# zhenyuw16/Uni3DETR

Hardware: AMD Instinct MI355X
Metric: scenes/sec (fwd+bwd) SUN-RGB-D 20k pts, 300 queries (higher is better)
Workload: dtype bf16

## Files before the change

include/u3d_hip.h:

```cpp
#ifndef U3D_HIP_H_
#define U3D_HIP_H_

#include <stddef.h>
#include <stdint.h>

#ifdef __cplusplus
extern "C" {
#endif

typedef struct ihipStream_t* u3d_stream;

enum {
  U3D_OK = 0,
  U3D_ERR_ARG = -1,
  U3D_ERR_UNSUPPORTED = -2,
  U3D_ERR_LAUNCH = -3,
  U3D_ERR_WORKSPACE = -4
};

enum { U3D_F32 = 0, U3D_BF16 = 1 };

int32_t u3d_version(void);
const char* u3d_strerror(int32_t code);

int32_t u3d_event_create(void** event);
int32_t u3d_event_record(void* event, int32_t external, u3d_stream s);
int32_t u3d_event_elapsed_ms(void* start, void* stop, float* ms);
int32_t u3d_event_destroy(void* event);

typedef struct u3d_bitgrid {
  void* words;
  void* prefix;
  int32_t batch, dz, dy, dx;
  int32_t layout;
  int32_t row_capacity;
} u3d_bitgrid;

int64_t u3d_bitgrid_nwords(int32_t batch, int32_t dz, int32_t dy, int32_t dx);
int64_t u3d_bitgrid_nwords_layout(int32_t batch, int32_t dz, int32_t dy, int32_t dx, int32_t layout);

int32_t u3d_bitgrid_mark(const u3d_bitgrid* g, const int32_t* coors, int32_t n, u3d_stream s);

int32_t u3d_bitgrid_mark_strided(const u3d_bitgrid* g, const int32_t* in_coors, const int32_t* n_dev,
                                 int32_t n_cap, const int32_t ksize[3], const int32_t stride[3],
                                 const int32_t pad[3], u3d_stream s);

int64_t u3d_bitgrid_scan_scratch(int64_t nwords);
int32_t u3d_bitgrid_scan(const u3d_bitgrid* g, void* scratch, u3d_stream s);

int32_t u3d_bitgrid_rank(const u3d_bitgrid* g, const int32_t* coors, int32_t n, int32_t* rank, u3d_stream s);

int32_t u3d_bitgrid_coords(const u3d_bitgrid* g, int32_t* coors_out, int32_t cap, u3d_stream s);

int32_t u3d_nbr_table(const u3d_bitgrid* target, const int32_t* q_coors, const int32_t* n_dev, int32_t n_cap,
                      const int32_t ksize[3], const int32_t stride[3], const int32_t pad[3], int32_t mode,
                      int32_t* nbr, int32_t ld, u3d_stream s);

int32_t u3d_dense_nbr_table(int32_t batch, const int32_t q_dims[3], const int32_t t_dims[3], const int32_t ksize[3],
                            const int32_t stride[3], const int32_t pad[3], int32_t mode, int32_t* nbr, int32_t ld,
                            u3d_stream s);

int64_t u3d_voxelize_hard_workspace(int32_t n_total, int32_t batch, int32_t max_pts_per_scene);
int32_t u3d_voxelize_hard(const float* points, const int32_t* scene_off, int32_t batch, int32_t n_total,
                          int32_t max_pts_per_scene, int32_t nfeat, const float voxel_size[3],
                          const float pc_range[6], int32_t max_points, int32_t max_voxels,
                          float* voxels, int32_t* coors, int32_t* num_points, float* mean,
                          int32_t* voxel_off, void* workspace, int64_t workspace_bytes, u3d_stream s);

int32_t u3d_voxelize_dynamic(const float* points, const int32_t* scene_off, int32_t batch, int32_t n_total, int32_t nfeat,
                             const float voxel_size[3], const float pc_range[6], int32_t* coors, u3d_stream s);
int32_t u3d_scatter_mean(const float* points, const int32_t* rank, int32_t n_total, int32_t nfeat, float* sums,
                         int32_t* counts, int32_t n_voxels, u3d_stream s);

int32_t u3d_spconv_fwd(const void* in, const void* w, const int32_t* nbr, int32_t ld, void* out,
                       const int32_t* n_out_dev, int32_t n_out_cap, int32_t cin, int32_t cout, int32_t kvol,
                       int32_t transpose_w, int32_t dtype, u3d_stream s);

int32_t u3d_igemm_fwd_bf16(const void* in, const void* w, const int32_t* nbr, int32_t ld, void* out,
                           const int32_t* n_out_dev, int32_t n_out_cap, int32_t cin, int32_t cout, int32_t kvol,
                           int32_t transpose_w, u3d_stream s);
int32_t u3d_igemm_fwd_add_bf16(const void* in, const void* w, const int32_t* nbr, int32_t ld, const void* addend, void* out,
                               const int32_t* n_out_dev, int32_t n_out_cap, int32_t cin, int32_t cout, int32_t kvol,
                               int32_t transpose_w, u3d_stream s);
int32_t u3d_linear_bf16(const void* x, const void* w, const float* bias, int32_t relu, void* out, const int32_t* m_dev,
                        int32_t m_cap, int32_t k, int32_t n, u3d_stream s);
int64_t u3d_bn_fold_job_bytes(void);
int32_t u3d_bn_fold_job_blocks(int32_t kvol, int32_t cout, int32_t cin);
int32_t u3d_bn_fold_batched(const void* jobs, int32_t njobs, int32_t total_blocks, u3d_stream s);
int32_t u3d_igemm_fwd_affine_bf16(const void* in, const void* w_folded, const int32_t* nbr, int32_t ld, const float* shift, int32_t relu,
                                  void* out, const int32_t* n_out_dev, int32_t n_out_cap, int32_t cin, int32_t cout, int32_t kvol,
                                  u3d_stream s);
int32_t u3d_igemm_fwd_affine_plan(int32_t n_out_cap, int32_t cin, int32_t cout, int32_t kvol, int32_t has_nbr, int32_t* kernel,
                                  int32_t* rows, int32_t* cols);
int32_t u3d_igemm_fwd_split_bf16(const void* in, const void* w, const int32_t* nbr, int32_t ld, float* out, const int32_t* n_out_dev,
                                 int32_t n_out_cap, int32_t cin, int32_t cout, int32_t kvol3, double* stats, const float* addend, u3d_stream s);
int32_t u3d_igemm_direct_split_bf16(const void* in, const void* w3, const int32_t* nbr, int32_t ld, float* out, const int32_t* n_out_dev,
                                    int32_t n_out_cap, int32_t n_in_cap, int32_t cin, int32_t cout, u3d_stream s);
int32_t u3d_igemm_direct_affine_bf16(const void* in, const void* w_folded, const int32_t* nbr, int32_t ld, const float* shift,
                                     int32_t relu, const void* addend, void* out, const int32_t* n_out_dev, int32_t n_out_cap,
                                     int32_t cin, int32_t cout, u3d_stream s);
// ... 468 lines not shown
```

uni3detr_amd/csrc/geometry.hip:

```cpp
#include "common.h"

extern "C" int64_t u3d_bitgrid_nwords(int32_t batch, int32_t dz, int32_t dy, int32_t dx) {
  return (int64_t)batch * ((dz + 3) / 4) * ((dy + 3) / 4) * ((dx + 3) / 4);
}
extern "C" int64_t u3d_bitgrid_nwords_layout(int32_t batch, int32_t dz, int32_t dy, int32_t dx, int32_t layout) {
  if (layout == 1) return ((int64_t)batch * dz * dy * dx + 63) / 64;
  return u3d_bitgrid_nwords(batch, dz, dy, dx);
}
static inline long long grid_nwords(const u3d_bitgrid* g) { return u3d_bitgrid_nwords_layout(g->batch, g->dz, g->dy, g->dx, g->layout); }

__global__ void k_bitgrid_mark(BitGridDev g, unsigned long long* words, const int4* __restrict__ coors, int n) {
  int i = blockIdx.x * blockDim.x + threadIdx.x;
  if (i >= n) return;
  int4 c = coors[i];
  if (c.x < 0 || c.x >= g.B) return;
  if ((unsigned)c.y >= (unsigned)g.Dz || (unsigned)c.z >= (unsigned)g.Dy || (unsigned)c.w >= (unsigned)g.Dx) return;
  atomicOr(&words[u3d_word_index(g, c.x, c.y, c.z, c.w)], 1ull << u3d_bit_index(g, c.x, c.y, c.z, c.w));
}

extern "C" int32_t u3d_bitgrid_mark(const u3d_bitgrid* g, const int32_t* coors, int32_t n, u3d_stream s) {
  U3D_REQUIRE(g && g->words && coors, U3D_ERR_ARG);
  if (n <= 0) return U3D_OK;
  BitGridDev d = u3d_make_grid(g);
  hipLaunchKernelGGL(k_bitgrid_mark, dim3(u3d_cdiv(n, 256)), dim3(256), 0, s, d, (unsigned long long*)g->words,
// ... 222 lines not shown
      int bit = __ffsll((long long)bits) - 1;
      bits &= bits - 1;
      long long t = w * 64 + bit;
      int x = (int)(t % g.Dx); t /= g.Dx;
      int y = (int)(t % g.Dy); t /= g.Dy;
      int z = (int)(t % g.Dz); t /= g.Dz;
      if ((int)r < cap) out[r] = make_int4((int)t, z, y, x);
      ++r;
    }
    return;
  }
  long long t = w;
  int bx = (int)(t % g.bx); t /= g.bx;
  int by = (int)(t % g.by); t /= g.by;
  int bz = (int)(t % g.bz); t /= g.bz;
  int b = (int)t;
  while (bits) {
    int bit = __ffsll((long long)bits) - 1;
    bits &= bits - 1;
    if ((int)r < cap) out[r] = make_int4(b, bz * 4 + (bit >> 4), by * 4 + ((bit >> 2) & 3), bx * 4 + (bit & 3));
    ++r;
  }
}

extern "C" int32_t u3d_bitgrid_coords(const u3d_bitgrid* g, int32_t* coors_out, int32_t cap, u3d_stream s) {
  U3D_REQUIRE(g && g->words && g->prefix && coors_out, U3D_ERR_ARG);
  long long nwords = grid_nwords(g);
  hipLaunchKernelGGL(k_bitgrid_coords, dim3(u3d_cdiv(nwords, 256)), dim3(256), 0, s, u3d_make_grid(g), nwords,
                     (int4*)coors_out, cap);
  U3D_CHECK_LAUNCH();
  return U3D_OK;
}

__global__ void k_nbr_table(BitGridDev g, const int4* __restrict__ q, const int* __restrict__ n_dev, int n_cap,
                            Conv3 cv, int mode, int* __restrict__ nbr, int ld) {
  int i = blockIdx.x * blockDim.x + threadIdx.x;
  if (i >= ld) return;
  int n = min(*n_dev, n_cap);
  int kvol = cv.k[0] * cv.k[1] * cv.k[2];
  if (i >= n) {
    for (int k = 0; k < kvol; ++k) nbr[(long long)k * ld + i] = -1;
    return;
  }
  int4 c = q[i];
  int k = 0;
  for (int kz = 0; kz < cv.k[0]; ++kz)
    for (int ky = 0; ky < cv.k[1]; ++ky)
      for (int kx = 0; kx < cv.k[2]; ++kx, ++k) {
        int r = -1;
        if (mode == 0) {
          r = u3d_grid_lookup(g, c.x, c.y * cv.s[0] - cv.p[0] + kz, c.z * cv.s[1] - cv.p[1] + ky, c.w * cv.s[2] - cv.p[2] + kx);
        } else {
          int tz = c.y + cv.p[0] - kz, ty = c.z + cv.p[1] - ky, tx = c.w + cv.p[2] - kx;
          if (tz >= 0 && ty >= 0 && tx >= 0 && tz % cv.s[0] == 0 && ty % cv.s[1] == 0 && tx % cv.s[2] == 0)
            r = u3d_grid_lookup(g, c.x, tz / cv.s[0], ty / cv.s[1], tx / cv.s[2]);
        }
        nbr[(long long)k * ld + i] = r;
      }
}

extern "C" int32_t u3d_nbr_table(const u3d_bitgrid* target, const int32_t* q_coors, const int32_t* n_dev, int32_t n_cap,
                                 const int32_t ksize[3], const int32_t stride[3], const int32_t pad[3], int32_t mode,
                                 int32_t* nbr, int32_t ld, u3d_stream s) {
  U3D_REQUIRE(target && target->words && target->prefix && q_coors && n_dev && nbr, U3D_ERR_ARG);
  U3D_REQUIRE(ld >= n_cap && (mode == 0 || mode == 1), U3D_ERR_ARG);
  if (ld <= 0) return U3D_OK;
  Conv3 cv;
  for (int i = 0; i < 3; ++i) { cv.k[i] = ksize[i]; cv.s[i] = stride[i]; cv.p[i] = pad[i]; U3D_REQUIRE(stride[i] > 0 && ksize[i] > 0, U3D_ERR_ARG); }
  hipLaunchKernelGGL(k_nbr_table, dim3(u3d_cdiv(ld, 256)), dim3(256), 0, s, u3d_make_grid(target), (const int4*)q_coors,
                     n_dev, n_cap, cv, mode, nbr, ld);
  U3D_CHECK_LAUNCH();
  return U3D_OK;
}

__global__ void k_dense_nbr_table(int B, int qz, int qy, int qx, int tz, int ty, int tx, Conv3 cv, int mode,
                                  int* __restrict__ nbr, int ld) {
  int i = blockIdx.x * blockDim.x + threadIdx.x;
  if (i >= ld) return;
  int kvol = cv.k[0] * cv.k[1] * cv.k[2];
  long long nq = (long long)B * qz * qy * qx;
  if (i >= nq) {
    for (int k = 0; k < kvol; ++k) nbr[(long long)k * ld + i] = -1;
    return;
  }
  int x = i % qx; int t = i / qx;
  int y = t % qy; t /= qy;
  int z = t % qz; int b = t / qz;
  int k = 0;
  for (int kz = 0; kz < cv.k[0]; ++kz)
    for (int ky = 0; ky < cv.k[1]; ++ky)
      for (int kx = 0; kx < cv.k[2]; ++kx, ++k) {
        int pz, py, px;
        bool ok = true;
        if (mode == 0) {
          pz = z * cv.s[0] - cv.p[0] + kz; py = y * cv.s[1] - cv.p[1] + ky; px = x * cv.s[2] - cv.p[2] + kx;
        } else {
          int uz = z + cv.p[0] - kz, uy = y + cv.p[1] - ky, ux = x + cv.p[2] - kx;
          ok = uz >= 0 && uy >= 0 && ux >= 0 && uz % cv.s[0] == 0 && uy % cv.s[1] == 0 && ux % cv.s[2] == 0;
          pz = uz / cv.s[0]; py = uy / cv.s[1]; px = ux / cv.s[2];
        }
        ok = ok && (unsigned)pz < (unsigned)tz && (unsigned)py < (unsigned)ty && (unsigned)px < (unsigned)tx;
        nbr[(long long)k * ld + i] = ok ? (int)((((long long)b * tz + pz) * ty + py) * tx + px) : -1;
      }
// ... 98 lines not shown
                           const int* __restrict__ slot_of, int* __restrict__ vid, int* __restrict__ scene_cnt) {
  __shared__ unsigned wsum[16];
  __shared__ unsigned carry_s;
  int b = blockIdx.x;
  int p0 = scene_off[b], n = scene_off[b + 1] - p0;
  long long tb = (long long)b * cfg.hsize;
  if (threadIdx.x == 0) carry_s = 0;
  __syncthreads();
  int lane = threadIdx.x & 63, wid = threadIdx.x >> 6;
  for (int base = 0; base < n; base += 1024) {
    int il = base + threadIdx.x;
    int sl = -1;
    unsigned flag = 0;
    if (il < n) {
      sl = slot_of[p0 + il];
      if (sl >= 0 && first[tb + sl] == (unsigned)il) flag = 1;
    }
    unsigned long long bal = __ballot(flag);
    unsigned in_wave = __popcll(bal & ((1ull << lane) - 1ull));
    if (lane == 0) wsum[wid] = __popcll(bal);
    __syncthreads();
    unsigned woff = 0, tot = 0;
    for (int w = 0; w < 16; ++w) { unsigned v = wsum[w]; if (w < wid) woff += v; tot += v; }
    unsigned carry = carry_s;
    if (flag) {
      unsigned r = carry + woff + in_wave;
      vid[tb + sl] = (r < (unsigned)cfg.max_voxels) ? (int)r : -1;
    }
    __syncthreads();
    if (threadIdx.x == 0) carry_s = carry + tot;
    __syncthreads();
  }
  if (threadIdx.x == 0) scene_cnt[b] = (int)min(carry_s, (unsigned)cfg.max_voxels);
}

__global__ void k_vox_offsets(const int* __restrict__ scene_cnt, int B, int* __restrict__ voxel_off) {
  if (threadIdx.x == 0 && blockIdx.x == 0) {
    int acc = 0;
    for (int b = 0; b < B; ++b) { voxel_off[b] = acc; acc += scene_cnt[b]; }
    voxel_off[B] = acc;
  }
}

__global__ void k_vox_write(const float* __restrict__ pts, const int* __restrict__ scene_off, int B, int n_total, VoxCfg cfg,
                            const unsigned* __restrict__ keys, const unsigned* __restrict__ first, const int* __restrict__ head,
                            const int* __restrict__ next, const int* __restrict__ slot_of, const int* __restrict__ vid,
                            const int* __restrict__ voxel_off, float* __restrict__ voxels, int4* __restrict__ coors,
                            int* __restrict__ num_points, float* __restrict__ mean) {
  int i = blockIdx.x * blockDim.x + threadIdx.x;
  if (i >= n_total || i >= scene_off[B]) return;
  int sl = slot_of[i];
  if (sl < 0) return;
  int b = 0;
  while (b + 1 < B && i >= scene_off[b + 1]) ++b;
  int p0 = scene_off[b];
  int il = i - p0;
  long long tb = (long long)b * cfg.hsize;
  if (first[tb + sl] != (unsigned)il) return;
  int v = vid[tb + sl];
  if (v < 0) return;
  long long row = (long long)voxel_off[b] + v;
  unsigned key = keys[tb + sl];
  int cx = (int)(key % (unsigned)cfg.grid[0]);
  unsigned t = key / (unsigned)cfg.grid[0];
  int cy = (int)(t % (unsigned)cfg.grid[1]);
  int cz = (int)(t / (unsigned)cfg.grid[1]);
// ... 2 lines not shown
  float acc[8];
  const int nf = cfg.nfeat;
  for (int f = 0; f < 8; ++f) acc[f] = 0.f;
  for (int r = 0; r < cfg.max_points; ++r) {
    int best = 0x7fffffff;
    for (int j = head[tb + sl]; j >= 0; j = next[p0 + j])
      if (j > last && j < best) best = j;
    if (best == 0x7fffffff) break;
    last = best;
    const float* p = pts + (long long)(p0 + best) * nf;
    for (int f = 0; f < nf; ++f) {
      float val = p[f];
      if (voxels) voxels[(row * cfg.max_points + r) * nf + f] = val;
      if (f < 8) acc[f] += val;
    }
    ++cnt;
  }
  if (voxels)
    for (int r = cnt; r < cfg.max_points; ++r)
      for (int f = 0; f < nf; ++f) voxels[(row * cfg.max_points + r) * nf + f] = 0.f;
  num_points[row] = cnt;
  if (mean) {
    float inv = (float)cnt;
    for (int f = 0; f < nf && f < 8; ++f) mean[row * nf + f] = acc[f] / inv;
  }
}

__global__ void k_fill_u32(unsigned* __restrict__ p, long long n, unsigned v) {
  for (long long i = (long long)blockIdx.x * blockDim.x + threadIdx.x; i < n; i += (long long)gridDim.x * blockDim.x) p[i] = v;
}

static inline int next_pow2(int v) { int p = 1; while (p < v) p <<= 1; return p; }

struct VoxWs { unsigned* keys; unsigned* first; int* head; int* vid; int* next; int* slot_of; int* scene_cnt; int hsize; int64_t bytes; };

static VoxWs vox_ws_layout(void* base, int n_total, int B, int max_pts_per_scene) {
  VoxWs w;
  w.hsize = next_pow2(2 * (max_pts_per_scene > 1 ? max_pts_per_scene : 1));
  char* p = (char*)base;
  size_t tab = (size_t)B * w.hsize * 4;
  w.keys = (unsigned*)p; p += tab;
  w.first = (unsigned*)p; p += tab;
  w.head = (int*)p; p += tab;
  w.vid = (int*)p; p += tab;
  w.next = (int*)p; p += (size_t)n_total * 4;
  w.slot_of = (int*)p; p += (size_t)n_total * 4;
  w.scene_cnt = (int*)p; p += (size_t)(B + 1) * 4;
  w.bytes = (int64_t)(p - (char*)base);
  return w;
}

extern "C" int64_t u3d_voxelize_hard_workspace(int32_t n_total, int32_t batch, int32_t max_pts_per_scene) {
  return vox_ws_layout(nullptr, n_total, batch, max_pts_per_scene).bytes;
}

extern "C" int32_t u3d_voxelize_hard(const float* points, const int32_t* scene_off, int32_t batch, int32_t n_total,
                                     int32_t max_pts_per_scene, int32_t nfeat, const float voxel_size[3],
                                     const float pc_range[6], int32_t max_points, int32_t max_voxels, float* voxels,
                                     int32_t* coors, int32_t* num_points, float* mean, int32_t* voxel_off,
                                     void* workspace, int64_t workspace_bytes, u3d_stream s) {
  U3D_REQUIRE(points && scene_off && coors && num_points && voxel_off && workspace, U3D_ERR_ARG);
  U3D_REQUIRE(batch > 0 && n_total >= 0 && nfeat >= 3 && nfeat <= 8 && max_points > 0 && max_voxels > 0, U3D_ERR_ARG);
  VoxWs w = vox_ws_layout(workspace, n_total, batch, max_pts_per_scene);
  U3D_REQUIRE(workspace_bytes >= w.bytes, U3D_ERR_WORKSPACE);
  VoxCfg cfg;
  for (int j = 0; j < 3; ++j) {
    cfg.vs[j] = voxel_size[j];
    cfg.lo[j] = pc_range[j];
    cfg.grid[j] = (int)lroundf((pc_range[3 + j] - pc_range[j]) / voxel_size[j]);
  }
  U3D_REQUIRE((long long)cfg.grid[0] * cfg.grid[1] * cfg.grid[2] < 0xFFFFFFFFll, U3D_ERR_ARG);
  cfg.nfeat = nfeat; cfg.max_points = max_points; cfg.max_voxels = max_voxels; cfg.hsize = w.hsize;
  {
    long long nfill = (long long)batch * w.hsize * 4;
    int blocks = (int)((nfill + 255) / 256); if (blocks > 2048) blocks = 2048;
    hipLaunchKernelGGL(k_fill_u32, dim3(blocks), dim3(256), 0, s, w.keys, nfill, 0xFFFFFFFFu);
  }
  if (n_total > 0) {
    hipLaunchKernelGGL(k_vox_insert, dim3(u3d_cdiv(n_total, 256)), dim3(256), 0, s, points, scene_off, batch, n_total, cfg,
                       w.keys, w.first, w.head, w.next, w.slot_of);
  }
  hipLaunchKernelGGL(k_vox_rank, dim3(batch), dim3(1024), 0, s, scene_off, cfg, (const unsigned*)w.first,
                     (const int*)w.slot_of, w.vid, w.scene_cnt);
  hipLaunchKernelGGL(k_vox_offsets, dim3(1), dim3(64), 0, s, (const int*)w.scene_cnt, batch, voxel_off);
  if (n_total > 0) {
    hipLaunchKernelGGL(k_vox_write, dim3(u3d_cdiv(n_total, 256)), dim3(256), 0, s, points, scene_off, batch, n_total, cfg,
                       (const unsigned*)w.keys, (const unsigned*)w.first, (const int*)w.head, (const int*)w.next,
                       (const int*)w.slot_of, (const int*)w.vid, (const int*)voxel_off, voxels, (int4*)coors, num_points, mean);
  }
  U3D_CHECK_LAUNCH();
  return U3D_OK;
}


__global__ void k_vox_dynamic(const float* __restrict__ pts, const int* __restrict__ scene_off, int B, int n_total, VoxCfg cfg,
                              int4* __restrict__ coors) {
  int i = blockIdx.x * blockDim.x + threadIdx.x;
  if (i >= n_total) return;
  int b = 0;
  while (b + 1 < B && i >= scene_off[b + 1]) ++b;
  const float* p = pts + (long long)i * cfg.nfeat;
  int c[3];
  bool ok = true;
#pragma unroll
  for (int j = 0; j < 3; ++j) {
    float q = __fdiv_rn(__fsub_rn(p[j], cfg.lo[j]), cfg.vs[j]);
    bool in = (q >= 0.f) && (q < (float)cfg.grid[j]);
    c[j] = in ? (int)floorf(q) : 0;
    ok = ok && in;
  }
  coors[i] = ok ? make_int4(b, c[2], c[1], c[0]) : make_int4(b, -1, -1, -1);
}

extern "C" int32_t u3d_voxelize_dynamic(const float* points, const int32_t* scene_off, int32_t batch, int32_t n_total, int32_t nfeat,
                                        const float voxel_size[3], const float pc_range[6], int32_t* coors, u3d_stream s) {
  U3D_REQUIRE(points && scene_off && coors && batch > 0 && nfeat >= 3, U3D_ERR_ARG);
  if (n_total <= 0) return U3D_OK;
  VoxCfg cfg;
  for (int j = 0; j < 3; ++j) {
    cfg.vs[j] = voxel_size[j];
    cfg.lo[j] = pc_range[j];
    cfg.grid[j] = (int)lroundf((pc_range[3 + j] - pc_range[j]) / voxel_size[j]);
  }
  cfg.nfeat = nfeat; cfg.max_points = 0; cfg.max_voxels = 0; cfg.hsize = 0;
  hipLaunchKernelGGL(k_vox_dynamic, dim3(u3d_cdiv(n_total, 256)), dim3(256), 0, s, points, scene_off, batch, n_total, cfg, (int4*)coors);
  U3D_CHECK_LAUNCH();
// ... 28 lines not shown
```

uni3detr_amd/native.py:

```python
import ctypes as C
import os

import numpy as np
import torch

from . import abi

_HERE = os.path.dirname(os.path.abspath(__file__))
LIB_PATH = os.environ.get("U3D_LIB_PATH") or os.path.join(_HERE, "libu3d_hip.so")

_ABI = abi.load()
_K = _ABI.constants


def _struct(c_name, py_name):
    return abi.structure(_ABI.structs[c_name], py_name)


def _slot_names(prefix):
    names = sorted((v, n[len(prefix):]) for n, v in _K.items() if n.startswith(prefix))
    assert [v for v, _ in names] == list(range(len(names))) and names[-1][1] == "COUNT" and _K[prefix + "COUNT"] == len(names) - 1
    return [n for _, n in names[:-1]]


# ... 73 lines not shown
        self.nwords = int(lib().u3d_bitgrid_nwords_layout(self.batch, *self.dims, 1 if linear else 0))
        self.words = torch.zeros(self.nwords, dtype=torch.int64, device=device)
        self.prefix = torch.empty(self.nwords + 1, dtype=torch.int32, device=device)
        self._scratch = torch.empty(int(lib().u3d_bitgrid_scan_scratch(self.nwords)), dtype=torch.int32, device=device)
        self.c = BitGridStruct(self.words.data_ptr(), self.prefix.data_ptr(), self.batch, *self.dims, 1 if linear else 0, 0)

    def set_row_capacity(self, cap):
        self.c.row_capacity = int(cap)

    def mark(self, coors):
        _check(lib().u3d_bitgrid_mark(C.byref(self.c), _ptr(coors), coors.shape[0], _stream()), "bitgrid_mark")

    def mark_strided(self, in_coors, n_dev, ksize, stride, pad):
        _check(lib().u3d_bitgrid_mark_strided(C.byref(self.c), _ptr(in_coors), _ptr(n_dev), in_coors.shape[0],
                                              _I3(*ksize), _I3(*stride), _I3(*pad), _stream()), "bitgrid_mark_strided")

    def scan(self):
        _check(lib().u3d_bitgrid_scan(C.byref(self.c), _ptr(self._scratch), _stream()), "bitgrid_scan")

    @property
    def count_dev(self):
        return self.prefix[self.nwords:]

    def rank(self, coors):
        out = torch.empty(coors.shape[0], dtype=torch.int32, device=coors.device)
        _check(lib().u3d_bitgrid_rank(C.byref(self.c), _ptr(coors), coors.shape[0], _ptr(out), _stream()), "bitgrid_rank")
        return out

    def coords(self, n):
        out = torch.empty((n, 4), dtype=torch.int32, device=self.words.device)
        _check(lib().u3d_bitgrid_coords(C.byref(self.c), _ptr(out), n, _stream()), "bitgrid_coords")
        return out

    def nbr_table(self, q_coors, n_dev, ksize, stride, pad, mode):
        n = q_coors.shape[0]
        ld = (n + 127) // 128 * 128
        kvol = ksize[0] * ksize[1] * ksize[2]
        nbr = torch.empty((kvol, ld), dtype=torch.int32, device=q_coors.device)
        _check(lib().u3d_nbr_table(C.byref(self.c), _ptr(q_coors), _ptr(n_dev), n, _I3(*ksize), _I3(*stride), _I3(*pad),
                                   mode, _ptr(nbr), ld, _stream()), "nbr_table")
        return nbr


def dense_nbr_table(batch, q_dims, t_dims, ksize, stride, pad, mode, device):
    n = batch * q_dims[0] * q_dims[1] * q_dims[2]
    ld = (n + 127) // 128 * 128
    kvol = ksize[0] * ksize[1] * ksize[2]
    nbr = torch.empty((kvol, ld), dtype=torch.int32, device=device)
    with torch.cuda.device(device):
        _check(lib().u3d_dense_nbr_table(batch, _I3(*q_dims), _I3(*t_dims), _I3(*ksize), _I3(*stride), _I3(*pad), mode, _ptr(nbr), ld,
                                         _stream()), "dense_nbr_table")
    return nbr


def voxelize_hard(points, scene_off, batch, max_pts_per_scene, voxel_size, pc_range, max_points, max_voxels,
                  want_voxels=True, want_mean=True):
    n_total, nfeat = points.shape
    cap = batch * max_voxels
    dev = points.device
    voxels = torch.empty((cap, max_points, nfeat), dtype=torch.float32, device=dev) if want_voxels else None
    coors = torch.full((cap, 4), -1, dtype=torch.int32, device=dev)
    num = torch.zeros((cap,), dtype=torch.int32, device=dev)
    mean = torch.zeros((cap, nfeat), dtype=torch.float32, device=dev) if want_mean else None
    voxel_off = torch.empty((batch + 1,), dtype=torch.int32, device=dev)
    wsb = int(lib().u3d_voxelize_hard_workspace(n_total, batch, max_pts_per_scene))
    ws = torch.empty(wsb, dtype=torch.uint8, device=dev)
    _check(lib().u3d_voxelize_hard(_ptr(points), _ptr(scene_off), batch, n_total, max_pts_per_scene, nfeat,
                                   _F3(*voxel_size), _F6(*pc_range), max_points, max_voxels, _ptr(voxels), _ptr(coors),
                                   _ptr(num), _ptr(mean), _ptr(voxel_off), _ptr(ws), wsb, _stream()), "voxelize_hard")
    return voxels, coors, num, mean, voxel_off


def voxelize_dynamic(points, scene_off, batch, voxel_size, pc_range):
    n_total, nfeat = points.shape
    coors = torch.empty((n_total, 4), dtype=torch.int32, device=points.device)
    _check(lib().u3d_voxelize_dynamic(_ptr(points), _ptr(scene_off), batch, n_total, nfeat, _F3(*voxel_size), _F6(*pc_range),
                                      _ptr(coors), _stream()), "voxelize_dynamic")
    return coors


def scatter_mean(points, rank, n_voxels):
    n_total, nfeat = points.shape
    sums = torch.zeros((n_voxels, nfeat), dtype=torch.float32, device=points.device)
    counts = torch.zeros((n_voxels,), dtype=torch.int32, device=points.device)
    _check(lib().u3d_scatter_mean(_ptr(points), _ptr(rank), n_total, nfeat, _ptr(sums), _ptr(counts), n_voxels, _stream()), "scatter_mean")
    return sums, counts


class ExternalEvent:

    def __init__(self):
        h = C.c_void_p()
        _check(lib().u3d_event_create(C.byref(h)), "event_create")
        self.h = h

    def record(self):
        _check(lib().u3d_event_record(self.h, 1, _stream()), "event_record")

    def elapsed_time(self, other):
        ms = C.c_float()
        _check(lib().u3d_event_elapsed_ms(self.h, other.h, C.byref(ms)), "event_elapsed_ms")
        return float(ms.value)
# ... 1845 lines not shown
```

uni3detr_amd/sparse.py:

```python
import collections
import contextlib
import os

import torch

from . import native as nv
from .shadow import conv_weights, halo_packs

K3, S1, P1 = (3, 3, 3), (1, 1, 1), (1, 1, 1)


class Level:

    def __init__(self, grid, coords, n, n_dev):
        self.grid, self.coords, self.n, self.n_dev = grid, coords, n, n_dev
        self.dims, self.batch = grid.dims, grid.batch
        self._subm = None
        self._halo = None

    def halo(self):
        if self._halo is None:
            h = nv.SubmHalo(self.subm_tables()[0], self.n_dev, self.n) if self.n <= nv.SubmHalo.MAX_ROWS else None
            self._halo = h if (h is not None and h.ok) else False
        return self._halo or None
# ... 25 lines not shown
        self.epi = nv.BnEpi.of(x, y, mean, invstd, gamma, beta, relu)
        self.c = x.shape[1]


class FanoutToken:

    def __init__(self, n):
        self.n = self.remaining = n
        self.acc = None

    def step(self, din):
        self.remaining -= 1
        if self.remaining > 0:
            self.acc = din
            return None
        self.acc, self.remaining = None, self.n
        return din


class ConvGeom:

    def __init__(self, nbr_fwd, nbr_bwd, n_in, n_in_dev, n_out, n_out_dev, kind="sparse", strided=False):
        self.strided = strided
        self.nbr_fwd, self.nbr_bwd = nbr_fwd, nbr_bwd
        self.n_in, self.n_in_dev, self.n_out, self.n_out_dev = n_in, n_in_dev, n_out, n_out_dev
        self.kind = kind
        self.level = None


def level_from_coors(coors, batch, dims):
    dev = coors.device
    g = nv.BitGrid(batch, dims, dev)
    g.mark(coors)
    g.scan()
    n = coors.shape[0]
    g.set_row_capacity(n)
    rank = g.rank(coors)
    lvl = Level(g, g.coords(n), n, g.count_dev)
    return lvl, rank


def subm_geom(lvl):
    fwd, bwd = lvl.subm_tables()
    g = ConvGeom(fwd, bwd, lvl.n, lvl.n_dev, lvl.n, lvl.n_dev)
    g.level = lvl
    return g


def strided_level(lvl, ksize, stride, pad, capacity=None):
    dims_out = tuple((d + 2 * p - k) // s + 1 for d, k, s, p in zip(lvl.dims, ksize, stride, pad))
    g = nv.BitGrid(lvl.batch, dims_out, lvl.coords.device)
    g.mark_strided(lvl.coords, lvl.n_dev, ksize, stride, pad)
    g.scan()
    n_out = int(g.count_dev.item()) if capacity is None else int(capacity)
    if capacity is not None:
        g.set_row_capacity(n_out)
    out = Level(g, g.coords(n_out), n_out, g.count_dev)
    fwd = lvl.grid.nbr_table(out.coords, out.n_dev, ksize, stride, pad, 0)
    bwd = g.nbr_table(lvl.coords, lvl.n_dev, ksize, stride, pad, 1)
    return out, ConvGeom(fwd, bwd, lvl.n, lvl.n_dev, n_out, out.n_dev, strided=True)


REV_SUBM_TABLE = True
SUBM_HALO = os.environ.get("U3D_SUBM_HALO", "1") == "1"
HALO_WGRAD = True
HALO_128 = True
STRIDED_DGRAD_SPLIT = True
NMAJOR_FWD = True
STRIDED_SPLIT_MIN_RATIO = 16
STRIDED_SPLIT_SPARSE_RATIO = 16


_CONV_USES = {}


def reset_conv_uses():
    _CONV_USES.clear()
    _PLANES_BWD.clear()


SPLIT_BF16 = os.environ.get("U3D_SPLIT_BF16", "1") == "1"
SPLIT_FUSED_ADD = True
_SPLIT = [False]


_PLANES = {}
_PLANES_BWD = {}
BN_PLANES = True


# ... 458 lines not shown
```

Before: 431.2.

## Fuse bitgrid scan with coord extraction, add k3 nbr-table kernel, chunk voxel ranking

Adds three independent geometry-preprocessing optimizations, all on by default. The bitgrid scan's final pass is fused with coordinate emission, removing a kernel launch and a reread of words and prefix. A specialized 3x3x3 neighbor-table kernel loads the 8 covering words and prefixes once per query instead of doing 27 separate lookups. Voxel ranking is split across chunked blocks per scene instead of one block per scene, and offsets are folded into the rank kernel. The costs are more register pressure in the fused scan, which keeps chunk sums per thread, and an extra counting pass in voxelization.

```diff
diff --git a/include/u3d_hip.h b/include/u3d_hip.h
--- a/include/u3d_hip.h
+++ b/include/u3d_hip.h
@@ -52,9 +52,14 @@
 
 int32_t u3d_bitgrid_coords(const u3d_bitgrid* g, int32_t* coors_out, int32_t cap, u3d_stream s);
 
+int32_t u3d_bitgrid_scan_coords(const u3d_bitgrid* g, void* scratch, int32_t* coors_out, int32_t cap, u3d_stream s);
+
 int32_t u3d_nbr_table(const u3d_bitgrid* target, const int32_t* q_coors, const int32_t* n_dev, int32_t n_cap,
                       const int32_t ksize[3], const int32_t stride[3], const int32_t pad[3], int32_t mode,
                       int32_t* nbr, int32_t ld, u3d_stream s);
+
+int32_t u3d_nbr_table_k3(const u3d_bitgrid* target, const int32_t* q_coors, const int32_t* n_dev, int32_t n_cap,
+                         const int32_t stride[3], const int32_t pad[3], int32_t mode, int32_t* nbr, int32_t ld, u3d_stream s);
 
 int32_t u3d_dense_nbr_table(int32_t batch, const int32_t q_dims[3], const int32_t t_dims[3], const int32_t ksize[3],
                             const int32_t stride[3], const int32_t pad[3], int32_t mode, int32_t* nbr, int32_t ld,
@@ -66,6 +71,11 @@
                           const float pc_range[6], int32_t max_points, int32_t max_voxels,
                           float* voxels, int32_t* coors, int32_t* num_points, float* mean,
                           int32_t* voxel_off, void* workspace, int64_t workspace_bytes, u3d_stream s);
+int32_t u3d_voxelize_hard_chunked(const float* points, const int32_t* scene_off, int32_t batch, int32_t n_total,
+                                  int32_t max_pts_per_scene, int32_t nfeat, const float voxel_size[3],
+                                  const float pc_range[6], int32_t max_points, int32_t max_voxels,
+                                  float* voxels, int32_t* coors, int32_t* num_points, float* mean,
+                                  int32_t* voxel_off, void* workspace, int64_t workspace_bytes, u3d_stream s);
 
 int32_t u3d_voxelize_dynamic(const float* points, const int32_t* scene_off, int32_t batch, int32_t n_total, int32_t nfeat,
                              const float voxel_size[3], const float pc_range[6], int32_t* coors, u3d_stream s);
diff --git a/uni3detr_amd/csrc/geometry.hip b/uni3detr_amd/csrc/geometry.hip
--- a/uni3detr_amd/csrc/geometry.hip
+++ b/uni3detr_amd/csrc/geometry.hip
@@ -278,6 +278,100 @@
   return U3D_OK;
 }
 
+#define SCAN_FUSED_MAX_CHUNKS 2048
+#define SCAN_FUSED_ONE_WORD_MAX (1 << 19)
+
+template <int ITEMS>
+__global__ __launch_bounds__(SCAN_TPB) void k_scan_final_coords(BitGridDev g, int nwords, const unsigned* __restrict__ chunk_sum,
+                                                                unsigned* __restrict__ prefix, int nchunks, int4* __restrict__ out,
+                                                                int cap) {
+  __shared__ unsigned lds[4];
+  __shared__ unsigned red[2][4];
+  const int lane = threadIdx.x & 63, wid = threadIdx.x >> 6;
+  const int sub0 = (int)blockIdx.x * (SCAN_TPB * ITEMS);
+  const int chunk = sub0 / SCAN_CHUNK;
+  const int base = sub0 + (int)threadIdx.x * ITEMS;
+  unsigned long long wd[ITEMS];
+  unsigned cs[SCAN_FUSED_MAX_CHUNKS / SCAN_TPB];
+  unsigned long long pw[SCAN_CHUNK / SCAN_TPB - ITEMS];
+#pragma unroll
+  for (int j = 0; j < ITEMS; ++j) wd[j] = g.words[min(base + j, nwords - 1)];
+#pragma unroll
+  for (int k = 0; k < SCAN_FUSED_MAX_CHUNKS / SCAN_TPB; ++k) cs[k] = chunk_sum[min(k * SCAN_TPB + (int)threadIdx.x, nchunks - 1)];
+#pragma unroll
+  for (int k = 0; k < SCAN_CHUNK / SCAN_TPB - ITEMS; ++k) {
+    const int wi = chunk * SCAN_CHUNK + k * SCAN_TPB + (int)threadIdx.x;
+    pw[k] = g.words[wi < sub0 ? wi : min(base, nwords - 1)];
+  }
+  unsigned before = 0, all = 0;
+#pragma unroll
+  for (int k = 0; k < SCAN_FUSED_MAX_CHUNKS / SCAN_TPB; ++k) {
+    const int ci = k * SCAN_TPB + (int)threadIdx.x;
+    all += (ci < nchunks) ? cs[k] : 0u;
+    before += (ci < chunk) ? cs[k] : 0u;
+  }
+#pragma unroll
+  for (int k = 0; k < SCAN_CHUNK / SCAN_TPB - ITEMS; ++k)
+    before += (chunk * SCAN_CHUNK + k * SCAN_TPB + (int)threadIdx.x < sub0) ? (unsigned)__popcll(pw[k]) : 0u;
+#pragma unroll
+  for (int o = 32; o > 0; o >>= 1) { before += __shfl_xor(before, o, 64); all += __shfl_xor(all, o, 64); }
+  if (lane == 0) { red[0][wid] = before; red[1][wid] = all; }
+  __syncthreads();
+  before = red[0][0] + red[0][1] + red[0][2] + red[0][3];
+  all = red[1][0] + red[1][1] + red[1][2] + red[1][3];
+
+  unsigned c = 0;
+#pragma unroll
+  for (int j = 0; j < ITEMS; ++j) {
+    if (base + j >= nwords) wd[j] = 0ull;
+    c += (unsigned)__popcll(wd[j]);
+  }
+  unsigned ex = block_exclusive_scan(c, lds, nullptr) + before;
+  if (blockIdx.x == 0 && threadIdx.x == 0) prefix[nwords] = all;
+  for (long long i = (long long)blockIdx.x * SCAN_TPB + threadIdx.x; i < cap; i += (long long)gridDim.x * SCAN_TPB)
+    if (i >= (long long)all) out[i] = make_int4(-1, -1, -1, -1);
+  int t = base;
+  int bx = t % g.bx; t /= g.bx;
+  int by = t % g.by; t /= g.by;
+  int bz = t % g.bz;
+  int b = t / g.bz;
+#pragma unroll
+  for (int j = 0; j < ITEMS; ++j) {
+    if (base + j < nwords) prefix[base + j] = ex;
+    unsigned long long bits = wd[j];
+    unsigned r = ex;
+    ex += (unsigned)__popcll(bits);
+    while (bits) {
+      const int bit = __ffsll((long long)bits) - 1;
+      bits &= bits - 1;
+      if (r < (unsigned)cap) out[r] = make_int4(b, bz * 4 + (bit >> 4), by * 4 + ((bit >> 2) & 3), bx * 4 + (bit & 3));
+      ++r;
+    }
+    if (++bx == g.bx) { bx = 0; if (++by == g.by) { by = 0; if (++bz == g.bz) { bz = 0; ++b; } } }
+  }
+}
+
+extern "C" int32_t u3d_bitgrid_scan_coords(const u3d_bitgrid* g, void* scratch, int32_t* coors_out, int32_t cap, u3d_stream s) {
+  U3D_REQUIRE(g && g->words && g->prefix && scratch && coors_out && cap >= 0, U3D_ERR_ARG);
+  const long long nwords = grid_nwords(g);
+  U3D_REQUIRE(nwords > 0, U3D_ERR_ARG);
+  const long long nchunks = (nwords + SCAN_CHUNK - 1) / SCAN_CHUNK;
+  if (g->layout != 0 || nchunks > SCAN_FUSED_MAX_CHUNKS) {
+    const int32_t rc = u3d_bitgrid_scan(g, scratch, s);
+    return rc != U3D_OK ? rc : u3d_bitgrid_coords(g, coors_out, cap, s);
+  }
+  unsigned* cs = (unsigned*)scratch;
+  hipLaunchKernelGGL(k_scan_chunksum, dim3((int)nchunks), dim3(SCAN_TPB), 0, s, (const unsigned long long*)g->words, nwords, cs);
+  if (nwords <= SCAN_FUSED_ONE_WORD_MAX)
+    hipLaunchKernelGGL(k_scan_final_coords<1>, dim3(u3d_cdiv(nwords, SCAN_TPB)), dim3(SCAN_TPB), 0, s, u3d_make_grid(g), (int)nwords,
+                       (const unsigned*)cs, (unsigned*)g->prefix, (int)nchunks, (int4*)coors_out, cap);
+  else
+    hipLaunchKernelGGL(k_scan_final_coords<4>, dim3(u3d_cdiv(nwords, SCAN_TPB * 4)), dim3(SCAN_TPB), 0, s, u3d_make_grid(g), (int)nwords,
+                       (const unsigned*)cs, (unsigned*)g->prefix, (int)nchunks, (int4*)coors_out, cap);
+  U3D_CHECK_LAUNCH();
+  return U3D_OK;
+}
+
 __global__ void k_nbr_table(BitGridDev g, const int4* __restrict__ q, const int* __restrict__ n_dev, int n_cap,
                             Conv3 cv, int mode, int* __restrict__ nbr, int ld) {
   int i = blockIdx.x * blockDim.x + threadIdx.x;
@@ -315,6 +409,117 @@
   for (int i = 0; i < 3; ++i) { cv.k[i] = ksize[i]; cv.s[i] = stride[i]; cv.p[i] = pad[i]; U3D_REQUIRE(stride[i] > 0 && ksize[i] > 0, U3D_ERR_ARG); }
   hipLaunchKernelGGL(k_nbr_table, dim3(u3d_cdiv(ld, 256)), dim3(256), 0, s, u3d_make_grid(target), (const int4*)q_coors,
                      n_dev, n_cap, cv, mode, nbr, ld);
+  U3D_CHECK_LAUNCH();
+  return U3D_OK;
+}
+
+template <int MODE>
+__device__ __forceinline__ void nbr_axis_k3(int c, int s, int p, int D, int nb, int (&t)[3], bool (&ok)[3], int (&blk)[2]) {
+  if (MODE == 0) {
+#pragma unroll
+    for (int j = 0; j < 3; ++j) { t[j] = c * s - p + j; ok[j] = (unsigned)t[j] < (unsigned)D; }
+  } else {
+    const int u0 = c + p;
+    const int q0 = u0 / s, r0 = u0 - q0 * s;
+#pragma unroll
+    for (int j = 0; j < 3; ++j) {
+      int r = (s == 1) ? 0 : r0 - j, q = (s == 1) ? u0 - j : q0;
+      if (r < 0) { r += s; q -= 1; }
+      t[j] = q;
+      ok[j] = u0 - j >= 0 && r == 0 && q < D;
+    }
+  }
+  int lo = 0x7fffffff;
+#pragma unroll
+  for (int j = 0; j < 3; ++j) if (ok[j]) lo = min(lo, t[j]);
+  blk[0] = (lo == 0x7fffffff) ? 0 : (lo >> 2);
+  blk[1] = min(blk[0] + 1, nb - 1);
+}
+
+template <int MODE>
+__global__ __launch_bounds__(256) void k_nbr_table_k3(BitGridDev g, const int4* __restrict__ q, const int* __restrict__ n_dev, int n_cap,
+                                                      Conv3 cv, int* __restrict__ nbr, int ld, int nwords) {
+  const int i = blockIdx.x * blockDim.x + threadIdx.x;
+  if (i >= ld) return;
+  const int n = min(*n_dev, n_cap);
+  if (i >= n) {
+#pragma unroll
+    for (int k = 0; k < 27; ++k) nbr[k * ld + i] = -1;
+    return;
+  }
+  const int4 c = q[i];
+  int tz[3], ty[3], tx[3], zb[2], yb[2], xb[2];
+  bool oz[3], oy[3], ox[3];
+  nbr_axis_k3<MODE>(c.y, cv.s[0], cv.p[0], g.Dz, g.bz, tz, oz, zb);
+  nbr_axis_k3<MODE>(c.z, cv.s[1], cv.p[1], g.Dy, g.by, ty, oy, yb);
+  nbr_axis_k3<MODE>(c.w, cv.s[2], cv.p[2], g.Dx, g.bx, tx, ox, xb);
+  int wi[2][2][2];
+#pragma unroll
+  for (int a = 0; a < 2; ++a)
+#pragma unroll
+    for (int b = 0; b < 2; ++b)
+#pragma unroll
+      for (int d = 0; d < 2; ++d)
+        wi[a][b][d] = (int)min((unsigned)(((c.x * g.bz + zb[a]) * g.by + yb[b]) * g.bx + xb[d]), (unsigned)(nwords - 1));
+  unsigned long long W[2][2][2];
+  unsigned P[2][2][2];
+#pragma unroll
+  for (int a = 0; a < 2; ++a)
+#pragma unroll
+    for (int b = 0; b < 2; ++b)
+#pragma unroll
+      for (int d = 0; d < 2; ++d) W[a][b][d] = g.words[wi[a][b][d]];
+#pragma unroll
+  for (int a = 0; a < 2; ++a)
+#pragma unroll
+    for (int b = 0; b < 2; ++b)
+#pragma unroll
+      for (int d = 0; d < 2; ++d) P[a][b][d] = g.prefix[wi[a][b][d]];
+#pragma unroll
+  for (int kz = 0; kz < 3; ++kz) {
+    const bool sz = (tz[kz] >> 2) != zb[0];
+    unsigned long long W4[2][2];
+    unsigned P4[2][2];
+#pragma unroll
+    for (int b = 0; b < 2; ++b)
+#pragma unroll
+      for (int d = 0; d < 2; ++d) { W4[b][d] = sz ? W[1][b][d] : W[0][b][d]; P4[b][d] = sz ? P[1][b][d] : P[0][b][d]; }
+#pragma unroll
+    for (int ky = 0; ky < 3; ++ky) {
+      const bool sy = (ty[ky] >> 2) != yb[0];
+      const unsigned long long W2[2] = {sy ? W4[1][0] : W4[0][0], sy ? W4[1][1] : W4[0][1]};
+      const unsigned P2[2] = {sy ? P4[1][0] : P4[0][0], sy ? P4[1][1] : P4[0][1]};
+#pragma unroll
+      for (int kx = 0; kx < 3; ++kx) {
+        const bool sx = (tx[kx] >> 2) != xb[0];
+        const unsigned long long bits = sx ? W2[1] : W2[0];
+        const unsigned pre = sx ? P2[1] : P2[0];
+        const int bit = ((tz[kz] & 3) << 4) | ((ty[ky] & 3) << 2) | (tx[kx] & 3);
+        const int r = (int)(pre + (unsigned)__popcll(bits & ((1ull << bit) - 1ull)));
+        const bool hit = (oz[kz] & oy[ky] & ox[kx]) & (bool)((bits >> bit) & 1ull) & !((g.cap > 0) & (r >= g.cap));
+        nbr[((kz * 3 + ky) * 3 + kx) * ld + i] = hit ? r : -1;
+      }
+    }
+  }
+}
+
+extern "C" int32_t u3d_nbr_table_k3(const u3d_bitgrid* target, const int32_t* q_coors, const int32_t* n_dev, int32_t n_cap,
+                                    const int32_t stride[3], const int32_t pad[3], int32_t mode, int32_t* nbr, int32_t ld,
+                                    u3d_stream s) {
+  U3D_REQUIRE(target && target->words && target->prefix && q_coors && n_dev && nbr, U3D_ERR_ARG);
+  U3D_REQUIRE(ld >= n_cap && (mode == 0 || mode == 1), U3D_ERR_ARG);
+  if (ld <= 0) return U3D_OK;
+  Conv3 cv;
+  for (int i = 0; i < 3; ++i) { cv.k[i] = 3; cv.s[i] = stride[i]; cv.p[i] = pad[i]; U3D_REQUIRE(stride[i] > 0, U3D_ERR_ARG); }
+  const long long nwords = grid_nwords(target);
+  U3D_REQUIRE(target->layout == 0 && pad[0] >= 0 && pad[1] >= 0 && pad[2] >= 0, U3D_ERR_UNSUPPORTED);
+  U3D_REQUIRE(nwords > 0 && nwords <= 0x7fffffffll && 27ll * ld <= 0x7fffffffll, U3D_ERR_UNSUPPORTED);
+  if (mode == 0)
+    hipLaunchKernelGGL(k_nbr_table_k3<0>, dim3(u3d_cdiv(ld, 256)), dim3(256), 0, s, u3d_make_grid(target), (const int4*)q_coors,
+                       n_dev, n_cap, cv, nbr, ld, (int)nwords);
+  else
+    hipLaunchKernelGGL(k_nbr_table_k3<1>, dim3(u3d_cdiv(ld, 256)), dim3(256), 0, s, u3d_make_grid(target), (const int4*)q_coors,
+                       n_dev, n_cap, cv, nbr, ld, (int)nwords);
   U3D_CHECK_LAUNCH();
   return U3D_OK;
 }
@@ -479,6 +684,86 @@
     __syncthreads();
   }
   if (threadIdx.x == 0) scene_cnt[b] = (int)min(carry_s, (unsigned)cfg.max_voxels);
+}
+
+#define VOX_CHUNK 1024
+
+__device__ __forceinline__ unsigned vox_creator_flags(const int* __restrict__ scene_off, int hsize, const unsigned* __restrict__ first,
+                                                      const int* __restrict__ slot_of, int b, int chunk, int& sl,
+                                                      unsigned& in_chunk_before, unsigned* wsum) {
+  const int p0 = scene_off[b], n = scene_off[b + 1] - p0;
+  const int il = chunk * VOX_CHUNK + (int)threadIdx.x;
+  const int lane = threadIdx.x & 63, wid = threadIdx.x >> 6;
+  sl = -1;
+  unsigned flag = 0;
+  if (il < n) {
+    sl = slot_of[p0 + il];
+    if (sl >= 0 && first[(long long)b * hsize + sl] == (unsigned)il) flag = 1;
+  }
+  const unsigned long long bal = __ballot(flag);
+  if (lane == 0) wsum[wid] = __popcll(bal);
+  __syncthreads();
+  unsigned woff = 0;
+  for (int w = 0; w < 16; ++w) woff += (w < wid) ? wsum[w] : 0u;
+  in_chunk_before = woff + __popcll(bal & ((1ull << lane) - 1ull));
+  return flag;
+}
+
+__global__ __launch_bounds__(VOX_CHUNK) void k_vox_chunk_count(const int* __restrict__ scene_off, int hsize,
+                                                               const unsigned* __restrict__ first, const int* __restrict__ slot_of,
+                                                               unsigned* __restrict__ chunk_cnt) {
+  __shared__ unsigned wsum[16];
+  int sl;
+  unsigned before;
+  vox_creator_flags(scene_off, hsize, first, slot_of, blockIdx.y, blockIdx.x, sl, before, wsum);
+  if (threadIdx.x == 0) {
+    unsigned tot = 0;
+    for (int w = 0; w < 16; ++w) tot += wsum[w];
+    chunk_cnt[blockIdx.y * gridDim.x + blockIdx.x] = tot;
+  }
+}
+
+__device__ __forceinline__ unsigned vox_wave_sum(unsigned v) {
+#pragma unroll
+  for (int o = 32; o > 0; o >>= 1) v += __shfl_xor(v, o, 64);
+  return v;
+}
+
+__global__ __launch_bounds__(VOX_CHUNK) void k_vox_rank_chunks(const int* __restrict__ scene_off, VoxCfg cfg, int B,
+                                                               const unsigned* __restrict__ first, const int* __restrict__ slot_of,
+                                                               const unsigned* __restrict__ chunk_cnt, int* __restrict__ vid,
+                                                               int* __restrict__ scene_cnt, int* __restrict__ voxel_off) {
+  __shared__ unsigned wsum[16];
+  __shared__ unsigned csum[16];
+  const int b = blockIdx.y, chunk = blockIdx.x, nchunk = gridDim.x;
+  const int lane = threadIdx.x & 63, wid = threadIdx.x >> 6;
+  unsigned carry = 0;
+  for (int j = threadIdx.x; j < chunk; j += VOX_CHUNK) carry += chunk_cnt[b * nchunk + j];
+  carry = vox_wave_sum(carry);
+  if (lane == 0) csum[wid] = carry;
+  int sl;
+  unsigned before;
+  const unsigned flag = vox_creator_flags(scene_off, cfg.hsize, first, slot_of, b, chunk, sl, before, wsum);
+  carry = 0;
+  for (int w = 0; w < 16; ++w) carry += csum[w];
+  if (flag) {
+    const unsigned r = carry + before;
+    vid[(long long)b * cfg.hsize + sl] = (r < (unsigned)cfg.max_voxels) ? (int)r : -1;
+  }
+  if (b == 0 && chunk == 0) {
+    for (int sb = wid; sb < B; sb += 16) {
+      unsigned tot = 0;
+      for (int j = lane; j < nchunk; j += 64) tot += chunk_cnt[sb * nchunk + j];
+      tot = vox_wave_sum(tot);
+      if (lane == 0) scene_cnt[sb] = (int)min(tot, (unsigned)cfg.max_voxels);
+    }
+    __syncthreads();
+    if (threadIdx.x == 0) {
+      int acc = 0;
+      for (int sb = 0; sb < B; ++sb) { voxel_off[sb] = acc; acc += scene_cnt[sb]; }
+      voxel_off[B] = acc;
+    }
+  }
 }
 
 __global__ void k_vox_offsets(const int* __restrict__ scene_cnt, int B, int* __restrict__ voxel_off) {
@@ -547,7 +832,7 @@
 
 static inline int next_pow2(int v) { int p = 1; while (p < v) p <<= 1; return p; }
 
-struct VoxWs { unsigned* keys; unsigned* first; int* head; int* vid; int* next; int* slot_of; int* scene_cnt; int hsize; int64_t bytes; };
+struct VoxWs { unsigned* keys; unsigned* first; int* head; int* vid; int* next; int* slot_of; int* scene_cnt; unsigned* chunk_cnt; int hsize; int nchunk; int64_t bytes; };
 
 static VoxWs vox_ws_layout(void* base, int n_total, int B, int max_pts_per_scene) {
   VoxWs w;
@@ -561,6 +846,8 @@
   w.next = (int*)p; p += (size_t)n_total * 4;
   w.slot_of = (int*)p; p += (size_t)n_total * 4;
   w.scene_cnt = (int*)p; p += (size_t)(B + 1) * 4;
+  w.nchunk = ((max_pts_per_scene > 1 ? max_pts_per_scene : 1) + VOX_CHUNK - 1) / VOX_CHUNK;
+  w.chunk_cnt = (unsigned*)p; p += (size_t)B * w.nchunk * 4;
   w.bytes = (int64_t)(p - (char*)base);
   return w;
 }
@@ -569,11 +856,11 @@
   return vox_ws_layout(nullptr, n_total, batch, max_pts_per_scene).bytes;
 }
 
-extern "C" int32_t u3d_voxelize_hard(const float* points, const int32_t* scene_off, int32_t batch, int32_t n_total,
-                                     int32_t max_pts_per_scene, int32_t nfeat, const float voxel_size[3],
-                                     const float pc_range[6], int32_t max_points, int32_t max_voxels, float* voxels,
-                                     int32_t* coors, int32_t* num_points, float* mean, int32_t* voxel_off,
-                                     void* workspace, int64_t workspace_bytes, u3d_stream s) {
+static int32_t voxelize_hard(const float* points, const int32_t* scene_off, int32_t batch, int32_t n_total,
+                             int32_t max_pts_per_scene, int32_t nfeat, const float voxel_size[3],
+                             const float pc_range[6], int32_t max_points, int32_t max_voxels, float* voxels,
+                             int32_t* coors, int32_t* num_points, float* mean, int32_t* voxel_off,
+                             void* workspace, int64_t workspace_bytes, bool chunk_ranks, u3d_stream s) {
   U3D_REQUIRE(points && scene_off && coors && num_points && voxel_off && workspace, U3D_ERR_ARG);
   U3D_REQUIRE(batch > 0 && n_total >= 0 && nfeat >= 3 && nfeat <= 8 && max_points > 0 && max_voxels > 0, U3D_ERR_ARG);
   VoxWs w = vox_ws_layout(workspace, n_total, batch, max_pts_per_scene);
@@ -595,9 +882,16 @@
     hipLaunchKernelGGL(k_vox_insert, dim3(u3d_cdiv(n_total, 256)), dim3(256), 0, s, points, scene_off, batch, n_total, cfg,
                        w.keys, w.first, w.head, w.next, w.slot_of);
   }
-  hipLaunchKernelGGL(k_vox_rank, dim3(batch), dim3(1024), 0, s, scene_off, cfg, (const unsigned*)w.first,
-                     (const int*)w.slot_of, w.vid, w.scene_cnt);
-  hipLaunchKernelGGL(k_vox_offsets, dim3(1), dim3(64), 0, s, (const int*)w.scene_cnt, batch, voxel_off);
+  if (chunk_ranks) {
+    hipLaunchKernelGGL(k_vox_chunk_count, dim3(w.nchunk, batch), dim3(VOX_CHUNK), 0, s, scene_off, w.hsize, (const unsigned*)w.first,
+                       (const int*)w.slot_of, w.chunk_cnt);
+    hipLaunchKernelGGL(k_vox_rank_chunks, dim3(w.nchunk, batch), dim3(VOX_CHUNK), 0, s, scene_off, cfg, batch,
+                       (const unsigned*)w.first, (const int*)w.slot_of, (const unsigned*)w.chunk_cnt, w.vid, w.scene_cnt, voxel_off);
+  } else {
+    hipLaunchKernelGGL(k_vox_rank, dim3(batch), dim3(1024), 0, s, scene_off, cfg, (const unsigned*)w.first,
+                       (const int*)w.slot_of, w.vid, w.scene_cnt);
+    hipLaunchKernelGGL(k_vox_offsets, dim3(1), dim3(64), 0, s, (const int*)w.scene_cnt, batch, voxel_off);
+  }
   if (n_total > 0) {
     hipLaunchKernelGGL(k_vox_write, dim3(u3d_cdiv(n_total, 256)), dim3(256), 0, s, points, scene_off, batch, n_total, cfg,
                        (const unsigned*)w.keys, (const unsigned*)w.first, (const int*)w.head, (const int*)w.next,
@@ -607,6 +901,22 @@
   return U3D_OK;
 }
 
+extern "C" int32_t u3d_voxelize_hard(const float* points, const int32_t* scene_off, int32_t batch, int32_t n_total,
+                                     int32_t max_pts_per_scene, int32_t nfeat, const float voxel_size[3],
+                                     const float pc_range[6], int32_t max_points, int32_t max_voxels, float* voxels,
+                                     int32_t* coors, int32_t* num_points, float* mean, int32_t* voxel_off,
+                                     void* workspace, int64_t workspace_bytes, u3d_stream s) {
+  return voxelize_hard(points, scene_off, batch, n_total, max_pts_per_scene, nfeat, voxel_size, pc_range, max_points, max_voxels, voxels,
+                       coors, num_points, mean, voxel_off, workspace, workspace_bytes, false, s);
+}
+extern "C" int32_t u3d_voxelize_hard_chunked(const float* points, const int32_t* scene_off, int32_t batch, int32_t n_total,
+                                             int32_t max_pts_per_scene, int32_t nfeat, const float voxel_size[3],
+                                             const float pc_range[6], int32_t max_points, int32_t max_voxels, float* voxels,
+                                             int32_t* coors, int32_t* num_points, float* mean, int32_t* voxel_off,
+                                             void* workspace, int64_t workspace_bytes, u3d_stream s) {
+  return voxelize_hard(points, scene_off, batch, n_total, max_pts_per_scene, nfeat, voxel_size, pc_range, max_points, max_voxels, voxels,
+                       coors, num_points, mean, voxel_off, workspace, workspace_bytes, true, s);
+}
 
 __global__ void k_vox_dynamic(const float* __restrict__ pts, const int* __restrict__ scene_off, int B, int n_total, VoxCfg cfg,
                               int4* __restrict__ coors) {
diff --git a/uni3detr_amd/native.py b/uni3detr_amd/native.py
--- a/uni3detr_amd/native.py
+++ b/uni3detr_amd/native.py
@@ -129,14 +129,32 @@
         _check(lib().u3d_bitgrid_coords(C.byref(self.c), _ptr(out), n, _stream()), "bitgrid_coords")
         return out
 
+    def scan_coords(self, n):
+        if not FUSED_SCAN_COORDS:
+            self.scan()
+            return self.coords(n)
+        out = torch.empty((n, 4), dtype=torch.int32, device=self.words.device)
+        _check(lib().u3d_bitgrid_scan_coords(C.byref(self.c), _ptr(self._scratch), _ptr(out), n, _stream()), "bitgrid_scan_coords")
+        return out
+
     def nbr_table(self, q_coors, n_dev, ksize, stride, pad, mode):
         n = q_coors.shape[0]
         ld = (n + 127) // 128 * 128
         kvol = ksize[0] * ksize[1] * ksize[2]
         nbr = torch.empty((kvol, ld), dtype=torch.int32, device=q_coors.device)
+        if (NBR_TABLE_K3 and tuple(ksize) == (3, 3, 3) and not self.linear and min(pad) >= 0 and self.nwords < 2 ** 31
+                and 27 * ld < 2 ** 31):
+            _check(lib().u3d_nbr_table_k3(C.byref(self.c), _ptr(q_coors), _ptr(n_dev), n, _I3(*stride), _I3(*pad), mode, _ptr(nbr), ld,
+                                          _stream()), "nbr_table_k3")
+            return nbr
         _check(lib().u3d_nbr_table(C.byref(self.c), _ptr(q_coors), _ptr(n_dev), n, _I3(*ksize), _I3(*stride), _I3(*pad),
                                    mode, _ptr(nbr), ld, _stream()), "nbr_table")
         return nbr
+
+
+NBR_TABLE_K3 = True
+FUSED_SCAN_COORDS = True
+VOX_CHUNK_RANKS = True
 
 
 def dense_nbr_table(batch, q_dims, t_dims, ksize, stride, pad, mode, device):
@@ -162,9 +180,10 @@
     voxel_off = torch.empty((batch + 1,), dtype=torch.int32, device=dev)
     wsb = int(lib().u3d_voxelize_hard_workspace(n_total, batch, max_pts_per_scene))
     ws = torch.empty(wsb, dtype=torch.uint8, device=dev)
-    _check(lib().u3d_voxelize_hard(_ptr(points), _ptr(scene_off), batch, n_total, max_pts_per_scene, nfeat,
-                                   _F3(*voxel_size), _F6(*pc_range), max_points, max_voxels, _ptr(voxels), _ptr(coors),
-                                   _ptr(num), _ptr(mean), _ptr(voxel_off), _ptr(ws), wsb, _stream()), "voxelize_hard")
+    fn = lib().u3d_voxelize_hard_chunked if VOX_CHUNK_RANKS else lib().u3d_voxelize_hard
+    _check(fn(_ptr(points), _ptr(scene_off), batch, n_total, max_pts_per_scene, nfeat,
+              _F3(*voxel_size), _F6(*pc_range), max_points, max_voxels, _ptr(voxels), _ptr(coors),
+              _ptr(num), _ptr(mean), _ptr(voxel_off), _ptr(ws), wsb, _stream()), "voxelize_hard")
     return voxels, coors, num, mean, voxel_off
 
 
diff --git a/uni3detr_amd/sparse.py b/uni3detr_amd/sparse.py
--- a/uni3detr_amd/sparse.py
+++ b/uni3detr_amd/sparse.py
@@ -81,11 +81,11 @@
     dev = coors.device
     g = nv.BitGrid(batch, dims, dev)
     g.mark(coors)
-    g.scan()
     n = coors.shape[0]
+    coords = g.scan_coords(n)
     g.set_row_capacity(n)
     rank = g.rank(coors)
-    lvl = Level(g, g.coords(n), n, g.count_dev)
+    lvl = Level(g, coords, n, g.count_dev)
     return lvl, rank
 
 
@@ -100,11 +100,15 @@
     dims_out = tuple((d + 2 * p - k) // s + 1 for d, k, s, p in zip(lvl.dims, ksize, stride, pad))
     g = nv.BitGrid(lvl.batch, dims_out, lvl.coords.device)
     g.mark_strided(lvl.coords, lvl.n_dev, ksize, stride, pad)
-    g.scan()
-    n_out = int(g.count_dev.item()) if capacity is None else int(capacity)
-    if capacity is not None:
+    if capacity is None:
+        g.scan()
+        n_out = int(g.count_dev.item())
+        coords = g.coords(n_out)
+    else:
+        n_out = int(capacity)
+        coords = g.scan_coords(n_out)
         g.set_row_capacity(n_out)
-    out = Level(g, g.coords(n_out), n_out, g.count_dev)
+    out = Level(g, coords, n_out, g.count_dev)
     fwd = lvl.grid.nbr_table(out.coords, out.n_dev, ksize, stride, pad, 0)
     bwd = g.nbr_table(lvl.coords, lvl.n_dev, ksize, stride, pad, 1)
     return out, ConvGeom(fwd, bwd, lvl.n, lvl.n_dev, n_out, out.n_dev, strided=True)
```

Result: faster. 437.1 (median of 6 runs) (+1.4%).
